# Alandroid/img-compression-mps

Hardware: AMD Instinct MI355X
Metric: Mvoxels/s compress+reconstruct, 256^3 fp32, bond chi=64; SSIM vs ref (higher is better)
Workload: dtype f32

## Files before the change

### img-compression-mps_amd/csrc/eig_tridiag.hip

```cpp
#include <math.h>
#include <stdlib.h>
#include <string.h>

#include <algorithm>
#include <atomic>
#include <map>
#include <mutex>
#include <vector>

#include "common.h"
#include "lanes.h"

namespace {
__device__ __forceinline__ double load_if(const double* p, bool ok) {
  const double v = *p;
  return ok ? v : 0.0;
}
}

namespace {

typedef double f64x4 __attribute__((ext_vector_type(4)));

constexpr int kTail = 128;
constexpr int kTailLd = 132;
constexpr int kMaxK = 128;
constexpr int kMaxN = 4096;

struct TrdDesc {
  const double* G_in;
  double* V_out;
  double* w_out;
  int n;
  int k;
  int status;
  int pad;
};

struct __attribute__((aligned(16))) TeamRec {
  double v;
  unsigned long long tag;
};

struct TeamSync {
  unsigned long long count;
  int abort;
  int pad[317];
};

struct TrdWork {
  double* A;
  double* Vh;
  double* y;
  double* xc;
  TeamRec* yr;
  TeamRec* xr;
  TeamSync* sync;
  double* tau;
  double* d;
  double* e;
  double* lam;
  double* mu;
  double* bound;
  double* Z;
  double* lu;
  unsigned char* piv;
  double* Tw;
  int64_t t_stride;
  double* yb;
  double* xb;
  double* band;
  double* qlog;
  int64_t q_stride;
  int tail_lower;
  int xcd_team, xcd_count;
  int xcd_pair;
  double* yrow;
  double* pv;
  double* pw;
  double* ypart;
  double* spart;
  double* ucol;
  double* napart;
  int pnl_blocks_max, pnl_tiles_max;
  long long* stamps;
  int n_max, lda, kp;
};

template <int STEPS>
__device__ __forceinline__ double fast_rsqrt(double x) {
  double y = __builtin_amdgcn_rsq(x);
#pragma unroll
  for (int i = 0; i < STEPS; ++i) y = y * fma(-0.5 * x * y, y, 1.5);
  return y;
}
template <int STEPS>
__device__ __forceinline__ double fast_rcp(double x) {
  double y = __builtin_amdgcn_rcp(x);
#pragma unroll
  for (int i = 0; i < STEPS; ++i) y = y * fma(-x, y, 2.0);
  return y;
}

__device__ __forceinline__ double wave_sum(double v) { return ndmps_lanes::sum_adjacent<64>(v); }

template <int NW>
// ... 18 lines not shown
  const double h2 = fma(alpha, alpha, sigma);
  const double rs = fast_rsqrt<2>(h2);
  const double nrm = h2 * rs;
  beta = alpha >= 0.0 ? -nrm : nrm;
  tau = (beta - alpha) * (alpha >= 0.0 ? -rs : rs);
  scale = fast_rcp<2>(alpha - beta);
}

__global__ void __launch_bounds__(256) trd_load_kernel(const TrdDesc* __restrict__ desc, TrdWork w) {
  const TrdDesc& d = desc[blockIdx.y];
  const int n = d.n, lda = w.lda;
  const double* G = d.G_in;
  double* A = w.A + (int64_t)blockIdx.y * w.n_max * lda;
  const int64_t total = (int64_t)n * lda;
  for (int64_t e = (int64_t)blockIdx.x * 256 + threadIdx.x; e < total; e += (int64_t)gridDim.x * 256) {
    const int r = (int)(e / lda), c = (int)(e % lda);
    A[e] = c < n ? 0.5 * (G[(int64_t)r * n + c] + G[(int64_t)c * n + r]) : 0.0;
  }
}

struct __attribute__((aligned(16))) RowVec {
  double vp, wp, vj, pad;
};

template <int NR, int CW>
__global__ void __launch_bounds__(256)
trd_column_kernel(const TrdDesc* __restrict__ desc, TrdWork w, int j) {
  constexpr int LPR = CW / 2;
  constexpr int RPW = 64 / LPR;
  constexpr int RPI = 4 * RPW;
  constexpr int PRE = 512 / RPI;
  const TrdDesc& d = desc[blockIdx.y];
  const int n = d.n;
  if (j >= n - kTail) return;
  const int c0 = blockIdx.x * CW;
  if (c0 >= n || c0 + CW <= j + 1) return;
  const int lda = w.lda;
  const int tid = threadIdx.x, lane = tid & 63, wave = tid >> 6;
  const int64_t b = blockIdx.y;
  double* A = w.A + b * w.n_max * lda;
  double* Vh = w.Vh + b * w.n_max * lda;
  double* ybuf = w.y + b * 2 * lda;
  extern __shared__ __attribute__((aligned(16))) double lds[];
  RowVec* rv = reinterpret_cast<RowVec*>(lds);
  __shared__ double red_a[4], red_b[4];
  __shared__ double part[4][CW];

  const int q = lane / LPR, p = lane % LPR;
  const int c = c0 + 2 * p;
  const bool col_ok = c < lda;
  const int first = j + 1 + RPW * wave + q;
  double2 a[PRE];
#pragma unroll
  for (int u = 0; u < PRE; ++u) {
    const int i = first + RPI * u;
    a[u] = (i < n && col_ok) ? *reinterpret_cast<const double2*>(A + (int64_t)i * lda + c) : make_double2(0.0, 0.0);
  }
  const double* rowj = A + (int64_t)j * lda;
  double yv[NR], vv[NR], rj[NR];
  double taup = 0.0, y_j = 0.0, y_j1 = 0.0, v_j1 = 0.0;
  const double r_j1 = rowj[j + 1];
  if (j >= 1) {
    const double* yprev = ybuf + ((j - 1) & 1) * lda;
    const double* vprev = Vh + (int64_t)(j - 1) * lda;
    taup = w.tau[b * w.n_max + j - 1];
    y_j = yprev[j];
    y_j1 = yprev[j + 1];
// ... 175 lines not shown
    member = blockIdx.x;
    team = blockIdx.y;
    return true;
  }
  const int L = blockIdx.x, full = w.xcd_count & ~7;
  if (L < full * w.xcd_team) {
    const int t = L >> 3;
    member = t % w.xcd_team;
    team = (t / w.xcd_team) * 8 + (L & 7);
    if (w.xcd_pair && ((t >> 5) & 1)) {
      const int blk = min(w.xcd_team, 32), pos = member % blk;
      member += blk - 1 - 2 * pos;
    }
  } else {
    const int r = w.xcd_count - full, l2 = L - full * w.xcd_team;
    member = l2 / r;
    team = full + l2 % r;
  }
  return true;
}

template <int NR, bool TAGGED, int CW = 32>
__global__ void __launch_bounds__(256, NR <= 4 ? 2 : 1)
trd_team_kernel(TrdDesc* __restrict__ desc, TrdWork w, int b0, unsigned epoch) {
  constexpr int MR = 256 * NR;
  constexpr int LPR = CW / 4;
  constexpr int RPW = 64 / LPR;
  constexpr int RPI = 4 * RPW;
  constexpr int NT = MR / RPI;
  int member, team;
  if (!team_place(w, member, team)) return;
  TrdDesc& d = desc[b0 + team];
  const int n = d.n;
  const int J = n - kTail;
  const int c0 = member * CW;
  if (J <= 0 || c0 >= n) return;
  const int nblk = (n + CW - 1) / CW;
  const int j_last = min(J - 1, c0 + CW - 2);
  const int lda = w.lda;
  const int tid = threadIdx.x, lane = tid & 63, wave = tid >> 6;
  const int64_t b = b0 + team;
  double* A = w.A + b * w.n_max * lda;
  double* Vh = w.Vh + b * w.n_max * lda;
  double* ybuf = w.y + b * 2 * lda;
  double* xc = w.xc + b * 2 * lda;
  TeamSync* sync = w.sync + b;
  TeamRec* yr = w.yr + b * 2 * lda;
  TeamRec* xr = w.xr + b * 2 * lda;
  const unsigned long long tag_base = (unsigned long long)epoch << 32;
  extern __shared__ __attribute__((aligned(32))) double team_dyn[];
  RowVec* rv = reinterpret_cast<RowVec*>(team_dyn);
  __shared__ double red_a[4], red_b[4];
  __shared__ double part[4][CW];
  __shared__ int go;

  const int q = lane % RPW, p = lane / RPW;
  const int c = c0 + 4 * p;
  const int row0 = RPW * wave + q;
  double a[NT][4];
#pragma unroll
  for (int u = 0; u < NT; ++u) {
    const int i = row0 + RPI * u;
    double2 lo = make_double2(0.0, 0.0), hi = lo;
    if (i < n) {
      if (c < lda) lo = *reinterpret_cast<const double2*>(A + (int64_t)i * lda + c);
      if (c + 2 < lda) hi = *reinterpret_cast<const double2*>(A + (int64_t)i * lda + c + 2);
    }
// ... 406 lines not shown
        sv.x -= me.vp * c0v.wp + me.wp * c0v.vp;
        sv.y -= me.vp * c1v.wp + me.wp * c1v.vp;
        acc = fma(sv.x, c0v.vj, acc);
        acc = fma(sv.y, c1v.vj, acc);
        *reinterpret_cast<double2*>(row + c) = sv;
      }
    }
    acc = ndmps_lanes::sum_adjacent<4>(acc);
    const double vjr = r < kTail ? cv[r].vj : 0.0;
    double dot = (t == 0 && r < m && r > jj) ? acc * vjr : 0.0;
    dot = wave_sum(dot);
    if (lane == 0) red_d[wave] = dot;
    __syncthreads();
    dot = 0.0;
#pragma unroll
    for (int x = 0; x < 8; ++x) dot += red_d[x];
    const double al = 0.5 * tau * tau * dot;
    if (t == 0 && r < m) {
      const double yr = r > jj ? acc : 0.0;
      cv[r].wp = tau * yr - al * vjr;
      cv[r].vp = vjr;
    }
    __syncthreads();
  }
  if (tid == 0) {
    const int jj = m - 1;
    dd[n - 1] = S[jj * kTailLd + jj] - 2.0 * cv[jj].vp * cv[jj].wp;
    ee[n - 1] = 0.0;
    tt[n - 1] = 0.0;
  }
  for (int i = tid; i < lda; i += 512) Vh[(int64_t)(n - 1) * lda + i] = 0.0;
}

__global__ void __launch_bounds__(512) trd_tail_reg_kernel(const TrdDesc* __restrict__ desc, TrdWork w) {
  const TrdDesc& d = desc[blockIdx.y];
  const int n = d.n;
  const int J = max(n - kTail, 0), m = n - J;
  const int lda = w.lda;
  const int tid = threadIdx.x, lane = tid & 63, wave = tid >> 6;
  const int64_t b = blockIdx.y;
  const double* A = w.A + b * w.n_max * lda;
  double* Vh = w.Vh + b * w.n_max * lda;
  const double* ybuf = w.y + b * 2 * lda;
  double* dd = w.d + b * w.n_max;
  double* ee = w.e + b * w.n_max;
  double* tt = w.tau + b * w.n_max;
  __shared__ RowVec cv[kTail];
  __shared__ double xrow[kTail];
  __shared__ double yv[kTail];
  __shared__ double red_s[8];

  for (int64_t e = tid; e < (int64_t)m * lda; e += 512) {
    const int i = (int)(e % lda);
    if (i < J || i >= n) Vh[(int64_t)J * lda + e] = 0.0;
  }
  if (J >= 1) {
    const double* yprev = ybuf + ((J - 1) & 1) * lda;
    const double* vprev = Vh + (int64_t)(J - 1) * lda;
    const double taup = tt[J - 1];
    double dot = 0.0, vv = 0.0, y0 = 0.0;
    if (tid < m) {
      vv = vprev[J + tid];
      y0 = yprev[J + tid];
      dot = y0 * vv;
    }
    dot = wave_sum(dot);
    if (lane == 0) red_s[wave] = dot;
    __syncthreads();
    dot = 0.0;
#pragma unroll
    for (int x = 0; x < 8; ++x) dot += red_s[x];
    const double al = 0.5 * taup * taup * dot;
    if (tid < kTail) {
      cv[tid].vp = tid < m ? vv : 0.0;
      cv[tid].wp = tid < m ? taup * y0 - al * vv : 0.0;
    }
  } else if (tid < kTail) {
    cv[tid].vp = 0.0;
    cv[tid].wp = 0.0;
  }
  __syncthreads();
  const int rg = tid >> 4, cg = tid & 15;
  double s[4][8];
#pragma unroll
  for (int a = 0; a < 4; ++a) {
    const int r = rg + 32 * a, gr = J + r;
    const double vpr = cv[r].vp, wpr = cv[r].wp;
#pragma unroll
    for (int q = 0; q < 8; ++q) {
      const int c = cg + 16 * q, gc = J + c;
      double v = 0.0;
      if (r < m && c < m) {
        const bool mirror = w.tail_lower && (gr >> 5) < (gc >> 5);
        const double av = mirror ? A[(int64_t)gc * lda + gr] : A[(int64_t)gr * lda + gc];
        v = av - (vpr * cv[c].wp + wpr * cv[c].vp);
      }
      s[a][q] = v;
    }
  }
  if (rg == 0) {
#pragma unroll
    for (int q = 0; q < 8; ++q) xrow[cg + 16 * q] = s[0][q];
  }
  __syncthreads();
  if (tid < kTail) {
    cv[tid].vp = 0.0;
    cv[tid].wp = 0.0;
    cv[tid].vj = 0.0;
  }
  __syncthreads();

  const int i0 = lane, i1 = lane + 64;
  double pv0 = 0.0, pv1 = 0.0, pw0 = 0.0, pw1 = 0.0;
  double tau_now = 0.0;
  auto pick = [&](double lo, double hi, int idx) {
    const double src = idx < 64 ? lo : hi;
    const long long bits = __double_as_longlong(src);
    const int l = __builtin_amdgcn_readlane((int)bits, idx & 63), h = __builtin_amdgcn_readlane((int)(bits >> 32), idx & 63);
    return __longlong_as_double(((long long)h << 32) | (unsigned)l);
  };
  for (int jj = 0; jj + 1 < m; ++jj) {
    const int j = J + jj;
    if (wave == 0) {
      const double vpj = pick(pv0, pv1, jj), wpj = pick(pw0, pw1, jj);
      double x0 = 0.0, x1 = 0.0;
      if (i0 < m) x0 = xrow[i0] - (vpj * pw0 + wpj * pv0);
      if (i1 < m) x1 = xrow[i1] - (vpj * pw1 + wpj * pv1);
      double sigma = (i0 > jj + 1 ? x0 * x0 : 0.0) + (i1 > jj + 1 ? x1 * x1 : 0.0);
      sigma = wave_sum(sigma);
      const double alpha = pick(x0, x1, jj + 1), djj = pick(x0, x1, jj);
      double beta, tau, scale;
      householder(alpha, sigma, beta, tau, scale);
      const double v0 = i0 > jj + 1 ? x0 * scale : (i0 == jj + 1 ? 1.0 : 0.0);
      const double v1 = i1 > jj + 1 ? x1 * scale : (i1 == jj + 1 ? 1.0 : 0.0);
      if (i0 < m) {
        cv[i0].vj = v0;
        Vh[(int64_t)j * lda + J + i0] = v0;
      }
      if (i1 < m) {
        cv[i1].vj = v1;
        Vh[(int64_t)j * lda + J + i1] = v1;
      }
      if (lane == 0) {
        dd[j] = djj;
        ee[j] = beta;
        tt[j] = tau;
      }
      tau_now = tau;
      pv0 = v0;
      pv1 = v1;
    }
    __syncthreads();
    double acc[4] = {0.0, 0.0, 0.0, 0.0};
    {
      const int q0 = (jj + 1) >> 4, a0 = (jj + 1) >> 5;
      double vpr[4], wpr[4];
#pragma unroll
      for (int a4 = 0; a4 < 4; ++a4) {
        vpr[a4] = cv[rg + 32 * a4].vp;
        wpr[a4] = cv[rg + 32 * a4].wp;
      }
#pragma unroll
      for (int h = 0; h < 2; ++h) {
        double vpc[4], wpc[4], vjc[4];
#pragma unroll
        for (int q = 0; q < 4; ++q) {
          const RowVec cr = cv[cg + 16 * (4 * h + q)];
          vpc[q] = cr.vp;
          wpc[q] = cr.wp;
          vjc[q] = cr.vj;
        }
#pragma unroll
        for (int a4 = 0; a4 < 4; ++a4) {
          if (a4 >= a0) {
#pragma unroll
            for (int q = 0; q < 4; ++q) {
              if (4 * h + q >= q0) {
                s[a4][4 * h + q] = fma(-vpr[a4], wpc[q], fma(-wpr[a4], vpc[q], s[a4][4 * h + q]));
                acc[a4] = fma(s[a4][4 * h + q], vjc[q], acc[a4]);
              }
            }
          }
        }
      }
      if (rg == ((jj + 1) & 31)) {
#define NDMPS_TAIL_PUT(AX) _Pragma("unroll") for (int q = 0; q < 8; ++q) xrow[cg + 16 * q] = s[AX][q];
        switch ((jj + 1) >> 5) {
          case 0: NDMPS_TAIL_PUT(0) break;
          case 1: NDMPS_TAIL_PUT(1) break;
          case 2: NDMPS_TAIL_PUT(2) break;
          default: NDMPS_TAIL_PUT(3) break;
        }
#undef NDMPS_TAIL_PUT
      }
    }
    const double y0 = ndmps_lanes::sum_adjacent<16>(acc[0]), y1 = ndmps_lanes::sum_adjacent<16>(acc[1]);
    const double y2 = ndmps_lanes::sum_adjacent<16>(acc[2]), y3 = ndmps_lanes::sum_adjacent<16>(acc[3]);
    if (cg < 4) {
      const int rr = rg + 32 * cg;
      const double yr = (cg & 2) ? ((cg & 1) ? y3 : y2) : ((cg & 1) ? y1 : y0);
      yv[rr] = rr > jj && rr < m ? yr : 0.0;
    }
    __syncthreads();
    if (wave == 0) {
      const double tau = tau_now;
      const double ya = yv[i0], yb = yv[i1];
      double dot = wave_sum(fma(ya, pv0, yb * pv1));
      const double al = 0.5 * tau * tau * dot;
      pw0 = tau * ya - al * pv0;
      pw1 = tau * yb - al * pv1;
      cv[i0].vp = pv0;
      cv[i0].wp = pw0;
      cv[i1].vp = pv1;
      cv[i1].wp = pw1;
    }
  }
  if (tid == 0) {
    const int jj = m - 1;
    dd[n - 1] = xrow[jj] - 2.0 * cv[jj].vp * cv[jj].wp;
    ee[n - 1] = 0.0;
    tt[n - 1] = 0.0;
  }
}

constexpr double kE2Floor = 0x1p-200;
__device__ __forceinline__ int sturm_count(const double2* __restrict__ de2, int n16, double x) {
  double pm = 0.0, pc = 1.0;
  int hp = 0;
  unsigned cnt = 0;
  for (int i0 = 0; i0 < n16; i0 += 16) {
    double2 v[16];
#pragma unroll
    for (int u = 0; u < 16; ++u) v[u] = de2[i0 + u];
#pragma unroll
    for (int u = 0; u < 16; ++u) {
      const double pn = fma(v[u].x - x, pc, -v[u].y * pm);
      const int hn = __double2hiint(pn);
      cnt += (unsigned)(hn ^ hp) >> 31;
      hp = hn;
      pm = pc;
      pc = pn;
      if ((u & 3) == 3) {
        const double mx = fmax(fabs(pm), fabs(pc));
        const int ex = mx > 0.0 ? ilogb(mx) : 0;
        pm = ldexp(pm, -ex);
        pc = ldexp(pc, -ex);
      }
// ... 899 lines not shown
    sync[base + t].abort = 0;
  }
}
__global__ void trd_setk_kernel(TrdDesc* __restrict__ desc, RankChunk chunk, int base, int count) {
  const int t = threadIdx.x;
  if (t < count) {
    desc[base + t].k = chunk.v[t];
    if (desc[base + t].status != 2) desc[base + t].status = 0;
  }
}
__global__ void trd_clear_status_kernel(TrdDesc* __restrict__ desc, int batch, TeamSync* __restrict__ sync) {
  const int b = blockIdx.x * blockDim.x + threadIdx.x;
  if (b < batch) {
    desc[b].status = 0;
    sync[b].count = 0;
    sync[b].abort = 0;
  }
}

#include "eig_band.inc"
#include "eig_sym.inc"
#include "eig_panel.inc"
#include "eig_wide.inc"

__global__ void trd_inject_abort_kernel(TrdDesc* __restrict__ desc, int batch) {
  const int b = blockIdx.x * blockDim.x + threadIdx.x;
  if (b < batch) desc[b].status = 2;
}

constexpr bool kTeamXcdDefault = true;
constexpr bool kSymDefault = false;
constexpr int kWideOrthoMinOrder = 1024;
constexpr int kWideOrthoMaxBatch = 2;
constexpr int kBandDefault = 0;

struct TrdLayout {
  int64_t n_max, lda, kp;
  int64_t off_a, off_vh, off_y, off_xc, off_yr, off_xr, off_sync, off_tau, off_d, off_e, off_lam, off_mu, off_bound, off_z, off_lu, off_piv, off_desc, off_desc2, off_stamps, off_tw, t_stride, off_yb, off_xb, off_band, off_qlog, q_stride, off_yrow, total;
  int64_t off_pv, off_pw, off_ypart, off_spart, off_ucol, off_napart, pnl_blocks, pnl_tiles;
  int64_t off_ws, off_wlinv, off_wgram, off_wt, wt_stride, kw, wgram_bytes, off_wpart, wpart_stride;
};

TrdLayout trd_layout(int64_t n_max, int64_t batch, int64_t k_max) {
  TrdLayout l;
  l.n_max = n_max;
  l.lda = ndmps::round_up(n_max, 2);
  l.kp = ndmps::round_up(std::max<int64_t>(k_max, 1), 16);
  int64_t used = 0;
  auto take = [&](int64_t bytes) {
    const int64_t off = ndmps::round_up(used, 256);
    used = off + bytes;
    return off;
  };
  l.off_a = take(batch * n_max * l.lda * 8);
  l.off_vh = take(batch * n_max * l.lda * 8);
  l.off_y = take(batch * 2 * l.lda * 8);
  l.off_xc = take(batch * 2 * l.lda * 8);
  l.off_yr = take(batch * 2 * l.lda * 16);
  l.off_xr = take(batch * 2 * l.lda * 16);
  l.off_sync = take(batch * (int64_t)sizeof(TeamSync));
  l.off_tau = take(batch * n_max * 8);
  l.off_d = take(batch * n_max * 8);
  l.off_e = take(batch * n_max * 8);
  l.off_lam = take(batch * n_max * 8);
  l.off_mu = take(batch * n_max * 8);
  l.off_bound = take(batch * 8);
// ... 42 lines not shown
  w.A = (double*)(base + l.off_a);
  w.Vh = (double*)(base + l.off_vh);
  w.y = (double*)(base + l.off_y);
  w.xc = (double*)(base + l.off_xc);
  w.yr = (TeamRec*)(base + l.off_yr);
  w.xr = (TeamRec*)(base + l.off_xr);
  w.sync = (TeamSync*)(base + l.off_sync);
  w.tau = (double*)(base + l.off_tau);
  w.d = (double*)(base + l.off_d);
  w.e = (double*)(base + l.off_e);
  w.lam = (double*)(base + l.off_lam);
  w.mu = (double*)(base + l.off_mu);
  w.bound = (double*)(base + l.off_bound);
  w.Z = (double*)(base + l.off_z);
  w.lu = (double*)(base + l.off_lu);
  w.piv = (unsigned char*)(base + l.off_piv);
  w.stamps = (long long*)(base + l.off_stamps);
  w.Tw = (double*)(base + l.off_tw);
  w.t_stride = l.t_stride;
  w.yb = (double*)(base + l.off_yb);
  w.xb = (double*)(base + l.off_xb);
  w.band = (double*)(base + l.off_band);
  w.qlog = (double*)(base + l.off_qlog);
  w.q_stride = l.q_stride;
  w.yrow = (double*)(base + l.off_yrow);
  w.pv = (double*)(base + l.off_pv);
  w.pw = (double*)(base + l.off_pw);
  w.ypart = (double*)(base + l.off_ypart);
  w.spart = (double*)(base + l.off_spart);
  w.ucol = (double*)(base + l.off_ucol);
  w.napart = (double*)(base + l.off_napart);
  w.pnl_blocks_max = (int)l.pnl_blocks;
  w.pnl_tiles_max = (int)l.pnl_tiles;
  w.tail_lower = 0;
  w.xcd_team = w.xcd_count = w.xcd_pair = 0;
  w.n_max = (int)l.n_max;
  w.lda = (int)l.lda;
  w.kp = (int)l.kp;
  return w;
}

constexpr int kInvitLdsMax = kMaxK * (kMaxK + 1) * 8;
constexpr size_t kTailLds = ((size_t)kTail * kTailLd + 4 * kTail) * sizeof(double);

thread_local int g_team_off = 0;
thread_local int g_team_streamed = 0;
std::atomic<long long> g_team_fallbacks{0};
std::atomic<int> g_inject_abort{0};


int trd_opt_in() {
  static std::mutex mu;
  static bool done[64] = {};
  int dev = 0;
  NDMPS_CHECK_HIP(hipGetDevice(&dev));
  std::lock_guard<std::mutex> lock(mu);
  if (dev < 0 || dev >= 64 || done[dev]) return NDMPS_OK;
  NDMPS_CHECK_HIP(hipFuncSetAttribute(reinterpret_cast<const void*>(&trd_tail_kernel),
                                      hipFuncAttributeMaxDynamicSharedMemorySize, (int)kTailLds));
  NDMPS_CHECK_HIP(hipFuncSetAttribute(reinterpret_cast<const void*>(&trd_team_kernel<8, true, 8>),
                                      hipFuncAttributeMaxDynamicSharedMemorySize, 2048 * (int)sizeof(RowVec)));
  NDMPS_CHECK_HIP(hipFuncSetAttribute(reinterpret_cast<const void*>(&trd_column_kernel<16, 32>),
                                      hipFuncAttributeMaxDynamicSharedMemorySize, kMaxN * (int)sizeof(RowVec)));
  NDMPS_CHECK_HIP(hipFuncSetAttribute(reinterpret_cast<const void*>(&trd_column_kernel<16, 8>),
                                      hipFuncAttributeMaxDynamicSharedMemorySize, kMaxN * (int)sizeof(RowVec)));
  NDMPS_CHECK_HIP(hipFuncSetAttribute(reinterpret_cast<const void*>(&trd_invit_kernel),
// ... 185 lines not shown
      const int nr = n_max <= 1024 ? 4 : 8;
      int slots = 0;
      NDMPS_TRY(team_slots(slots, nr));
      const int team_size = (int)ndmps::ceil_div(n_max, 8);
      const int per_launch = std::max(1, slots / team_size);
      w.tail_lower = 0;
      int inject = g_inject_abort.load();
      while (inject > 0 && !g_inject_abort.compare_exchange_weak(inject, inject - 1)) {
      }
      if (inject > 0) {
        hipLaunchKernelGGL(trd_inject_abort_kernel, dim3((batch + 63) / 64), dim3(64), 0, s, desc, batch);
        return NDMPS_OK;
      }
      return team_launch(s, [&]() {
        for (int b0 = 0; b0 < batch; b0 += per_launch) {
          const unsigned epoch = g_team_epoch.fetch_add(1);
          const dim3 grid((unsigned)team_size, (unsigned)std::min(per_launch, batch - b0));
          TrdWork wl = w;
          wl.xcd_count = 0;
          if (nr == 4) hipLaunchKernelGGL((trd_team_kernel<4, true, 8>), grid, dim3(256), 1024 * sizeof(RowVec), s, desc, wl, b0, epoch);
          else hipLaunchKernelGGL((trd_team_kernel<8, true, 8>), grid, dim3(256), 2048 * sizeof(RowVec), s, desc, wl, b0, epoch);
        }
      });
    }
    int slots = 0;
    NDMPS_TRY(team_slots(slots));
    const bool streamed = g_team_streamed && !getenv("NDMPS_TRD_TEAM_NARROW");
    const bool narrow_team = (int64_t)batch * ndmps::ceil_div(n_max, 8) <= (streamed ? slots / 2 : slots) &&
                             !getenv("NDMPS_TRD_TEAM_WIDE");
    const char* sym_env = getenv("NDMPS_TRD_SYM");
    const bool sym = !narrow_team && n_max <= 512 && (sym_env ? atoi(sym_env) != 0 : kSymDefault) &&
                     (int64_t)batch * ndmps::ceil_div(n_max, 32) > slots / 2;
    w.tail_lower = sym ? 1 : 0;
    const int team_size = sym ? (int)ndmps::ceil_div(ndmps::ceil_div(n_max, 32), 2) : (int)ndmps::ceil_div(n_max, narrow_team ? 8 : 32);
    const bool half_launches = getenv("NDMPS_TRD_TEAM_HALF") != nullptr && !narrow_team && !sym;
    const int per_launch = std::max(1, (half_launches ? slots / 2 : slots) / team_size);
    const char* xcd_env = getenv("NDMPS_TRD_XCD");
    const bool xcd_placed = xcd_env ? atoi(xcd_env) != 0 : kTeamXcdDefault;
    int inject = g_inject_abort.load();
    while (inject > 0 && !g_inject_abort.compare_exchange_weak(inject, inject - 1)) {
    }
    if (inject > 0) {
      hipLaunchKernelGGL(trd_inject_abort_kernel, dim3((batch + 63) / 64), dim3(64), 0, s, desc, batch);
    } else
    NDMPS_TRY(team_launch(s, [&]() {
      for (int b0 = 0; b0 < batch; b0 += per_launch) {
        const unsigned epoch = g_team_epoch.fetch_add(1);
        const int count = std::min(per_launch, batch - b0);
        TrdWork wl = w;
        dim3 grid((unsigned)team_size, (unsigned)count);
        if (xcd_placed) {
          wl.xcd_team = team_size;
          wl.xcd_count = count;
          const bool pairable = 32 % team_size == 0 || team_size % 32 == 0;
          wl.xcd_pair = sym || !pairable ? 0 : getenv("NDMPS_TRD_PAIR") ? atoi(getenv("NDMPS_TRD_PAIR")) : 1;
          grid = dim3((unsigned)(team_size * count));
        }
        if (sym) hipLaunchKernelGGL(trd_sym_kernel, grid, dim3(256), 0, s, desc, wl, b0);
        else if (narrow_team) hipLaunchKernelGGL((trd_team_kernel<2, true, 8>), grid, dim3(256), 512 * sizeof(RowVec), s, desc, wl, b0, epoch);
        else hipLaunchKernelGGL((trd_team_kernel<2, false>), grid, dim3(256), 512 * sizeof(RowVec), s, desc, wl, b0, epoch);
      }
    }, (int64_t)std::min(per_launch, batch) * team_size <= slots / 2));
  return NDMPS_OK;
}

int trd_reduce_and_values(int batch, const int64_t* h_n, int64_t n_max, int64_t k_max, const TrdLayout& l, const TrdWork& w_in,
                          TrdDesc* desc, hipStream_t s) {
  TrdWork w = w_in;
  const unsigned B = (unsigned)batch;
  const int load_grid = (int)std::min<int64_t>(ndmps::ceil_div(n_max * l.lda, 256), 512);
  hipLaunchKernelGGL(trd_load_kernel, dim3(load_grid, B), dim3(256), 0, s, desc, w);
  const bool narrow = (int64_t)batch * ndmps::ceil_div(n_max, 8) <= 2 * ndmps::kNumCU && !getenv("NDMPS_TRD_WIDE");
  const int W = (int)ndmps::ceil_div(n_max, narrow ? 8 : 32);
  const size_t col_lds = (size_t)n_max * sizeof(RowVec);
  void (*column)(const TrdDesc*, TrdWork, int);
  if (narrow)
    column = n_max <= 512    ? trd_column_kernel<2, 8>
             : n_max <= 1024 ? trd_column_kernel<4, 8>
             : n_max <= 2048 ? trd_column_kernel<8, 8>
                             : trd_column_kernel<16, 8>;
  else
    column = n_max <= 512    ? trd_column_kernel<2, 32>
             : n_max <= 1024 ? trd_column_kernel<4, 32>
             : n_max <= 2048 ? trd_column_kernel<8, 32>
                             : trd_column_kernel<16, 32>;
  const int bw = band_width_for(n_max);
  route_store(w_in.A, bw);
  const bool team = !bw && n_max <= 512 && n_max > kTail && !getenv("NDMPS_TRD_NO_TEAM") && !g_team_off;
  if (bw) {
    int slots = 0;
    NDMPS_TRY(team_slots(slots));
    const int team_size = (int)ndmps::ceil_div(n_max, 32);
    const int per_launch = std::max(1, slots / team_size);
    int inject = g_inject_abort.load();
    while (inject > 0 && !g_inject_abort.compare_exchange_weak(inject, inject - 1)) {
    }
    void* span = ndmps::span_begin(s);
    if (inject > 0) {
      hipLaunchKernelGGL(trd_inject_abort_kernel, dim3((batch + 63) / 64), dim3(64), 0, s, desc, batch);
    } else {
      NDMPS_TRY(team_launch(s, [&]() {
        for (int b0 = 0; b0 < batch; b0 += per_launch) {
          const dim3 grid((unsigned)team_size, (unsigned)std::min(per_launch, batch - b0));
          if (bw == 2) hipLaunchKernelGGL(trd_band_kernel<2>, grid, dim3(256), 0, s, desc, w, b0);
          else hipLaunchKernelGGL(trd_band_kernel<4>, grid, dim3(256), 0, s, desc, w, b0);
        }
      }));
    }
    int64_t bytes = 0;
    for (int b = 0; b < batch; ++b) bytes += 2 * 8 * h_n[b] * h_n[b];
    ndmps::span_end(span, s, ndmps::kSpanTridiagTeam, 1, bytes);
    const size_t chase_lds = (size_t)n_max * 2 * bw * sizeof(double);
    if (bw == 2) hipLaunchKernelGGL(trd_chase_kernel<2>, dim3(1, B), dim3(1024), chase_lds, s, desc, w);
    else hipLaunchKernelGGL(trd_chase_kernel<4>, dim3(1, B), dim3(1024), chase_lds, s, desc, w);
    const int kk = (int)std::min(k_max, n_max);
    hipLaunchKernelGGL(trd_bisect_kernel, dim3(ndmps::ceil_div(kk, 4), B), dim3(256),
                       (size_t)ndmps::round_up(n_max, 16) * 16, s, desc, w, kk);
    NDMPS_LAUNCH_CHECK();
    return NDMPS_OK;
  }
  const bool team_on = !bw && !g_team_off && !getenv("NDMPS_TRD_NO_TEAM");
// ... 49 lines not shown
    }
    NDMPS_TRY(pnl_run(seq, batch, h_n, n_max, tail_cols, desc, w, s));
    if (hybrid) {
      const int64_t J0 = n_max - hybrid;
      TrdDesc* sub = (TrdDesc*)((char*)w_in.A - l.off_a + l.off_desc2);
      hipLaunchKernelGGL(pnl_mirror_kernel, dim3(256, B), dim3(256), 0, s, w, (int)n_max, hybrid);
      hipLaunchKernelGGL(pnl_subdesc_kernel, dim3((batch + 63) / 64), dim3(64), 0, s, (const TrdDesc*)desc, sub, batch, hybrid);
      TrdWork v = w;
      v.A = w.A + J0 * l.lda + J0;
      v.Vh = w.Vh + J0 * l.lda + J0;
      v.y = w.y + J0;
      v.tau = w.tau + J0;
      v.d = w.d + J0;
      v.e = w.e + J0;
      NDMPS_TRY(trd_team_reduce(batch, hybrid, sub, v, s));
      hipLaunchKernelGGL(pnl_substatus_kernel, dim3((batch + 63) / 64), dim3(64), 0, s, desc, (const TrdDesc*)sub, batch);
      w.tail_lower = 0;
    } else {
      NDMPS_CHECK_HIP(hipMemsetAsync(w.y, 0, (size_t)batch * 2 * l.lda * 8, s));
    }
    ndmps::span_end(span, s, ndmps::kSpanTridiagPanel, (int64_t)seq.size(), span_bytes);
  } else {
    for (int j = 0; j < n_max - kTail; ++j) {
      hipLaunchKernelGGL(column, dim3(W, B), dim3(256), col_lds, s, desc, w, j);
      if (span)
        for (int b = 0; b < batch; ++b)
          if (j < h_n[b] - kTail) span_bytes += 2 * 8 * (h_n[b] - j - 1) * (h_n[b] - j - 1);
    }
    ndmps::span_end(span, s, ndmps::kSpanTridiagColumns, std::max<int64_t>(n_max - kTail, 0), span_bytes);
  }
  const char* tail_env = getenv("NDMPS_TRD_TAIL");
  const bool tail_regs = tail_env ? !strcmp(tail_env, "regs") : batch < 16;
  void* tail_span = ndmps::span_begin(s);
  if (tail_regs) hipLaunchKernelGGL(trd_tail_reg_kernel, dim3(1, B), dim3(512), 0, s, desc, w);
  else hipLaunchKernelGGL(trd_tail_kernel, dim3(1, B), dim3(512), kTailLds, s, desc, w);
  const int kk = (int)std::min(k_max, n_max);
  hipLaunchKernelGGL(trd_bisect_kernel, dim3(ndmps::ceil_div(kk, 4), B), dim3(256),
                     (size_t)ndmps::round_up(n_max, 16) * 16, s, desc, w, kk);
  ndmps::span_end(tail_span, s, ndmps::kSpanTridiagTail, 2, 0);
  NDMPS_LAUNCH_CHECK();
  return NDMPS_OK;
}

}

extern "C" int64_t ndmps_potrf_scratch_elems(int64_t n) {
  const int64_t kw = ndmps::round_up(std::max<int64_t>(n, 1), kWB);
  return kw * kw + 64;
}
extern "C" int ndmps_potrf_lower_f64(double* d_S, int64_t n, double* d_scratch, int* h_status, ndmps_stream_t stream) {
  NDMPS_REQUIRE(d_S && d_scratch && h_status && n >= 1 && n <= 32768, "bad Cholesky argument");
  NDMPS_TRY(trd_opt_in());
  hipStream_t s = (hipStream_t)stream;
  const int k = (int)n, kw = (int)ndmps::round_up(n, kWB), nblk = kw / kWB;
  double* linv = d_scratch;
  TrdDesc* d_flag = reinterpret_cast<TrdDesc*>(d_scratch + (int64_t)kw * kw);
  NDMPS_CHECK_HIP(hipMemsetAsync(d_flag, 0, sizeof(TrdDesc), s));
  for (int pb = 0; pb < nblk; ++pb) {
    const int p = kWB * pb, below = nblk - pb - 1;
    hipLaunchKernelGGL(wide_chol_diag_kernel, dim3(1), dim3(512), (size_t)2 * kWB * kWLd * sizeof(double), s, d_S, k, linv, kw, k, p,
                       d_flag);
    if (below > 0) {
      hipLaunchKernelGGL(wide_chol_panel_kernel, dim3((unsigned)below), dim3(256), 0, s, d_S, k, (const double*)linv, kw, k, p);
      hipLaunchKernelGGL(wide_chol_trail_kernel, dim3((unsigned)(below * (below + 1) / 2)), dim3(256), 0, s, d_S, k, k, p);
    }
  }
  hipLaunchKernelGGL(wide_zero_upper_kernel, dim3((unsigned)std::min<int64_t>(ndmps::ceil_div(n * n, 256), 2048)), dim3(256), 0, s,
// ... 348 lines not shown
```

### img-compression-mps_amd/csrc/tt.hip

```cpp
#include <math.h>
#include <stdlib.h>

#include <algorithm>
#include <vector>

#include "common.h"
#include "trunc.h"

namespace {

constexpr double kCutoffFloor = 1e-6;
constexpr double kCutoffFloorF64 = 1e-8;
template <typename T>
constexpr double cutoff_floor() { return sizeof(T) == 8 ? kCutoffFloorF64 : kCutoffFloor; }
constexpr double kSweepEigTol = 1e-13;

inline double sweep_eig_tol(bool f64_storage = false) {
  const char* e = getenv("NDMPS_SWEEP_EIG_TOL");
  if (e) {
    const double v = atof(e);
    if (v >= 1e-16 && v <= 1e-6) return v;
  }
  return f64_storage ? 1e-15 : kSweepEigTol;
}
// ... 97 lines not shown
scale_cols_to_f32_kernel(const double* __restrict__ M, int64_t rows, int64_t ldm, int64_t k,
                         const double* __restrict__ sigma, double power, T* __restrict__ out) {
  scale_cols_body(M, rows, ldm, k, sigma, power, out);
}
template <typename T>
__global__ void __launch_bounds__(256)
scale_rows_to_f32_kernel(const double* __restrict__ M, int64_t k, int64_t n, const double* __restrict__ sigma,
                         double power, T* __restrict__ out) {
  scale_rows_body(M, k, n, sigma, power, out);
}
__global__ void __launch_bounds__(256) sqrt_clamp_kernel(const double* __restrict__ w, int64_t n, double* s) {
  sqrt_clamp_body(w, n, s);
}

__global__ void __launch_bounds__(256)
scale_cols_sqrt_kernel(double* __restrict__ M, int64_t rows, int64_t cols, const double* __restrict__ w,
                       double rel_zero = 0.0) {
  const double zero = rel_zero * fmax(fmax(w[0], w[cols - 1]), 0.0);
  const int64_t total = rows * cols;
  for (int64_t e = (int64_t)blockIdx.x * 256 + threadIdx.x; e < total; e += (int64_t)gridDim.x * 256) {
    const double we = w[e % cols];
    M[e] *= we > zero ? sqrt(we) : 0.0;
  }
}

constexpr int kSmallBatch = 64;
struct BatchOps {
  const void* in[kSmallBatch];
  void* out[kSmallBatch];
};
template <typename T>
__global__ void __launch_bounds__(256) f32_to_f64_batched_kernel(BatchOps ops, int64_t n, double* __restrict__ y, int64_t y_stride) {
  f32_to_f64_body(static_cast<const T*>(ops.in[blockIdx.y]), n, y + (int64_t)blockIdx.y * y_stride);
}
template <typename T>
__global__ void __launch_bounds__(256)
core_from_vectors_batched_kernel(const double* __restrict__ V, int64_t v_stride, int64_t n, int64_t k, BatchOps ops) {
  core_from_vectors_body(V + (int64_t)blockIdx.y * v_stride, n, k, static_cast<T*>(ops.out[blockIdx.y]));
}
__global__ void __launch_bounds__(256)
sqrt_clamp_batched_kernel(const double* __restrict__ w, int64_t stride, int64_t n, double* __restrict__ sg) {
  sqrt_clamp_body(w + (int64_t)blockIdx.y * stride, n, sg + (int64_t)blockIdx.y * stride);
}
template <typename T>
__global__ void __launch_bounds__(256)
scale_cols_to_f32_batched_kernel(const double* __restrict__ M, int64_t m_stride, int64_t rows, int64_t ldm, int64_t k,
                                 const double* __restrict__ sigma, int64_t s_stride, double power, BatchOps ops) {
  scale_cols_body(M + (int64_t)blockIdx.y * m_stride, rows, ldm, k, sigma + (int64_t)blockIdx.y * s_stride, power,
                  static_cast<T*>(ops.out[blockIdx.y]));
}
template <typename T>
__global__ void __launch_bounds__(256)
scale_rows_to_f32_batched_kernel(const double* __restrict__ M, int64_t m_stride, int64_t k, int64_t n,
                                 const double* __restrict__ sigma, int64_t s_stride, double power, BatchOps ops) {
  scale_rows_body(M + (int64_t)blockIdx.y * m_stride, k, n, sigma + (int64_t)blockIdx.y * s_stride, power,
                  static_cast<T*>(ops.out[blockIdx.y]));
}

struct MergeRanks {
  int k_right[64];
  int k_here[64];
};

__global__ void __launch_bounds__(256)
merge_stage1_kernel(const double* __restrict__ Gtop, int64_t stride_top, int n_top, const double* __restrict__ W,
                    int64_t stride_w, int ldw, double* __restrict__ T, int64_t stride_t, int n_i, int n_right,
// ... 871 lines not shown
    hipLaunchKernelGGL(scale_cols_to_f32_batched_kernel<T>, dim3(grid1d(m * k), batch), dim3(256), 0, s, ws.V,
                       sq, m, m, k, ws.sig, lay.small_max, 1.0, carry_out);
    NDMPS_LAUNCH_CHECK();
    NDMPS_TRY(ndmps_dgemm_batched(batch, 1, 0, k, n, m, pv.data(), m, pa.data(), n, pu.data(), n, s));
    hipLaunchKernelGGL(scale_rows_to_f32_batched_kernel<T>, dim3(grid1d(k * n), batch), dim3(256), 0, s,
                       ws.UtA, lay.wide_elems, k, n, ws.sig, lay.small_max, -1.0,
                       cores_out);
    NDMPS_LAUNCH_CHECK();
    return NDMPS_OK;
  }

  int core_and_carry_volume(int i, int b) {
    const int64_t n = h_dims[i] * chi_r[b], m = cur_elems[b] / n, small = eig_n[b], k = kept[b];
    const double* sigb = ws.sig + (int64_t)b * lay.small_max;
    if (n <= m) {
      hipLaunchKernelGGL(core_from_vectors_kernel<T>, dim3(grid1d(k * n)), dim3(256), 0, s, Vb(b), n, k,
                         core(b, i));
      NDMPS_LAUNCH_CHECK();
      return gemm_T(1, m, k, n, cur[b], core(b, i), n, nxt[b], ws.tws, lay.transpose_bytes, s);
    }
    hipLaunchKernelGGL(sqrt_clamp_kernel, dim3(grid1d(small)), dim3(256), 0, s, ws.w + (int64_t)b * lay.small_max,
                       small, ws.sig + (int64_t)b * lay.small_max);
    hipLaunchKernelGGL(scale_cols_to_f32_kernel<T>, dim3(grid1d(m * k)), dim3(256), 0, s, Vb(b), m, m, k, sigb,
                       1.0, nxt[b]);
    NDMPS_LAUNCH_CHECK();
    NDMPS_TRY(ndmps_dgemm(1, 0, k, n, m, Vb(b), m, ws.A64 + (int64_t)b * lay.wide_elems, n, ws.UtA, n, s));
    hipLaunchKernelGGL(scale_rows_to_f32_kernel<T>, dim3(grid1d(k * n)), dim3(256), 0, s, ws.UtA, k, n, sigb,
                       -1.0, core(b, i));
    NDMPS_LAUNCH_CHECK();
    return NDMPS_OK;
  }

  int finish() {
    for (int b = 0; b < batch; ++b)
      NDMPS_CHECK_HIP(hipMemcpyAsync(core(b, 0), cur[b], cur_elems[b] * sizeof(T), hipMemcpyDeviceToDevice, s));
    if (!lay.device_rank || L <= 1) {
      if (async) {
        ndmps::set_error("an asynchronous sweep needs ranks decided on the device (ndmps_tt_sweep_pads_cores) and more than one site");
        return NDMPS_EINVAL;
      }
      NDMPS_CHECK_HIP(hipStreamSynchronize(s));
      return NDMPS_OK;
    }
    const size_t n_i = (size_t)2 * L * batch, n_s = (size_t)L * batch * lay.spec_stride;
    std::vector<int> host_i(async ? 0 : n_i);
    std::vector<double> host_s(async ? 0 : n_s);
    if (async) NDMPS_REQUIRE(async->h_ranks && (async->h_spec || n_s == 0), "asynchronous sweep without its host buffers");
    int* dst_i = async ? async->h_ranks : host_i.data();
    double* dst_s = async ? async->h_spec : host_s.data();
    NDMPS_CHECK_HIP(hipMemcpyAsync(dst_i, ws.d_ranks, n_i * sizeof(int), hipMemcpyDeviceToHost, s));
    if (n_s) NDMPS_CHECK_HIP(hipMemcpyAsync(dst_s, ws.d_spec, n_s * sizeof(double), hipMemcpyDeviceToHost, s));
    if (async) return NDMPS_OK;
    NDMPS_CHECK_HIP(hipStreamSynchronize(s));
    return sweep_collect(batch, L, lay.spec_stride, dst_i, n_s ? dst_s : nullptr, h_bonds_out, h_spectra, h_spec_offsets);
  }
};

template <typename T>
int sweep_impl(int batch, T* const* h_dense, int L, const int64_t* h_dims, double cutoff, int64_t max_bond,
               T* const* h_cores, const int64_t* h_core_offsets, int64_t* h_bonds_out, double* h_spectra,
               const int64_t* h_spec_offsets, void* d_ws, int64_t ws_bytes, ndmps_stream_t stream,
               const SweepSource* src = nullptr, const SweepAsync* async = nullptr) {
  Sweep<T> sw{batch, h_dense, L, h_dims, cutoff, max_bond, h_cores, h_core_offsets, h_bonds_out, h_spectra,
              h_spec_offsets, d_ws, ws_bytes, (hipStream_t)stream, src, async};
  NDMPS_TRY(sw.prepare());
  int i = L - 1;
  if (sw.lay.merge_from < L) {
    NDMPS_TRY(sw.merged_run());
// ... 747 lines not shown
```

Measured before the change: 42440.

## Template tail tridiagonal kernel on order and batch final core copies

The register-resident tail tridiagonalization kernel is templated on the trailing order (128 or 192), with a runtime tail width in the work struct. The wider tail is selected only when the NDMPS_TRD_TAIL_COLS environment variable asks for it. Separately, the per-batch device-to-device memcpy calls in finish() are replaced by one batched copy kernel launch per 64 items, which cuts launch and API overhead. The tail kernel also now reads previous v/w from shared memory instead of registers, which may add shared-memory traffic.

Measured after the change: 42510, median of 3. Within noise of the previous version (+0.2%).

```diff
diff --git a/img-compression-mps_amd/csrc/eig_tridiag.hip b/img-compression-mps_amd/csrc/eig_tridiag.hip
--- a/img-compression-mps_amd/csrc/eig_tridiag.hip
+++ b/img-compression-mps_amd/csrc/eig_tridiag.hip
@@ -23,6 +23,7 @@
 typedef double f64x4 __attribute__((ext_vector_type(4)));
 
 constexpr int kTail = 128;
+constexpr int kTailWide = 192;
 constexpr int kTailLd = 132;
 constexpr int kMaxK = 128;
 constexpr int kMaxN = 4096;
@@ -72,6 +73,7 @@
   double* band;
   double* qlog;
   int64_t q_stride;
+  int tail;
   int tail_lower;
   int xcd_team, xcd_count;
   int xcd_pair;
@@ -156,7 +158,7 @@
   constexpr int PRE = 512 / RPI;
   const TrdDesc& d = desc[blockIdx.y];
   const int n = d.n;
-  if (j >= n - kTail) return;
+  if (j >= n - w.tail) return;
   const int c0 = blockIdx.x * CW;
   if (c0 >= n || c0 + CW <= j + 1) return;
   const int lda = w.lda;
@@ -398,7 +400,7 @@
   if (!team_place(w, member, team)) return;
   TrdDesc& d = desc[b0 + team];
   const int n = d.n;
-  const int J = n - kTail;
+  const int J = n - w.tail;
   const int c0 = member * CW;
   if (J <= 0 || c0 >= n) return;
   const int nblk = (n + CW - 1) / CW;
@@ -871,10 +873,17 @@
   for (int i = tid; i < lda; i += 512) Vh[(int64_t)(n - 1) * lda + i] = 0.0;
 }
 
-__global__ void __launch_bounds__(512) trd_tail_reg_kernel(const TrdDesc* __restrict__ desc, TrdWork w) {
+template <int M>
+__global__ void __launch_bounds__(4 * M) trd_tail_reg_kernel(const TrdDesc* __restrict__ desc, TrdWork w) {
+  static_assert(M == 128 || M == 192, "trailing order 128 or 192");
+  constexpr int NTH = 4 * M;
+  constexpr int RB = M / 4;
+  constexpr int NQ = M / 16;
+  constexpr int NP = M / 64;
+  constexpr int NWV = NTH / 64;
   const TrdDesc& d = desc[blockIdx.y];
   const int n = d.n;
-  const int J = max(n - kTail, 0), m = n - J;
+  const int J = max(n - M, 0), m = n - J;
   const int lda = w.lda;
   const int tid = threadIdx.x, lane = tid & 63, wave = tid >> 6;
   const int64_t b = blockIdx.y;
@@ -884,14 +893,14 @@
   double* dd = w.d + b * w.n_max;
   double* ee = w.e + b * w.n_max;
   double* tt = w.tau + b * w.n_max;
-  __shared__ RowVec cv[kTail];
-  __shared__ double xrow[kTail];
-  __shared__ double yv[kTail];
-  __shared__ double red_s[8];
-
-  for (int64_t e = tid; e < (int64_t)m * lda; e += 512) {
+  __shared__ RowVec cv[M];
+  __shared__ double xrow[M];
+  __shared__ double yv[M];
+  __shared__ double red_s[NWV];
+
+  for (int64_t e = tid; e < (int64_t)m * lda; e += NTH) {
     const int i = (int)(e % lda);
-    if (i < J || i >= n) Vh[(int64_t)J * lda + e] = 0.0;
+    if (i < J || i >= n || e >= (int64_t)(m - 1) * lda) Vh[(int64_t)J * lda + e] = 0.0;
   }
   if (J >= 1) {
     const double* yprev = ybuf + ((J - 1) & 1) * lda;
@@ -908,25 +917,25 @@
     __syncthreads();
     dot = 0.0;
 #pragma unroll
-    for (int x = 0; x < 8; ++x) dot += red_s[x];
+    for (int x = 0; x < NWV; ++x) dot += red_s[x];
     const double al = 0.5 * taup * taup * dot;
-    if (tid < kTail) {
+    if (tid < M) {
       cv[tid].vp = tid < m ? vv : 0.0;
       cv[tid].wp = tid < m ? taup * y0 - al * vv : 0.0;
     }
-  } else if (tid < kTail) {
+  } else if (tid < M) {
     cv[tid].vp = 0.0;
     cv[tid].wp = 0.0;
   }
   __syncthreads();
   const int rg = tid >> 4, cg = tid & 15;
-  double s[4][8];
+  double s[4][NQ];
 #pragma unroll
   for (int a = 0; a < 4; ++a) {
-    const int r = rg + 32 * a, gr = J + r;
+    const int r = rg + RB * a, gr = J + r;
     const double vpr = cv[r].vp, wpr = cv[r].wp;
 #pragma unroll
-    for (int q = 0; q < 8; ++q) {
+    for (int q = 0; q < NQ; ++q) {
       const int c = cg + 16 * q, gc = J + c;
       double v = 0.0;
       if (r < m && c < m) {
@@ -939,46 +948,49 @@
   }
   if (rg == 0) {
 #pragma unroll
-    for (int q = 0; q < 8; ++q) xrow[cg + 16 * q] = s[0][q];
+    for (int q = 0; q < NQ; ++q) xrow[cg + 16 * q] = s[0][q];
   }
   __syncthreads();
-  if (tid < kTail) {
+  if (tid < M) {
     cv[tid].vp = 0.0;
     cv[tid].wp = 0.0;
     cv[tid].vj = 0.0;
   }
   __syncthreads();
 
-  const int i0 = lane, i1 = lane + 64;
-  double pv0 = 0.0, pv1 = 0.0, pw0 = 0.0, pw1 = 0.0;
   double tau_now = 0.0;
-  auto pick = [&](double lo, double hi, int idx) {
-    const double src = idx < 64 ? lo : hi;
+  auto pick3 = [](double x0, double x1, double x2, int idx) {
+    double src = (idx >> 6) == 1 ? x1 : x0;
+    if constexpr (NP > 2) src = (idx >> 6) == 2 ? x2 : src;
     const long long bits = __double_as_longlong(src);
     const int l = __builtin_amdgcn_readlane((int)bits, idx & 63), h = __builtin_amdgcn_readlane((int)(bits >> 32), idx & 63);
     return __longlong_as_double(((long long)h << 32) | (unsigned)l);
   };
+  auto pick = [&](const double (&x)[NP], int idx) { return pick3(x[0], x[1], x[NP - 1], idx); };
   for (int jj = 0; jj + 1 < m; ++jj) {
     const int j = J + jj;
     if (wave == 0) {
-      const double vpj = pick(pv0, pv1, jj), wpj = pick(pw0, pw1, jj);
-      double x0 = 0.0, x1 = 0.0;
-      if (i0 < m) x0 = xrow[i0] - (vpj * pw0 + wpj * pv0);
-      if (i1 < m) x1 = xrow[i1] - (vpj * pw1 + wpj * pv1);
-      double sigma = (i0 > jj + 1 ? x0 * x0 : 0.0) + (i1 > jj + 1 ? x1 * x1 : 0.0);
+      const double vpj = cv[jj].vp, wpj = cv[jj].wp;
+      double x[NP];
+      double sigma = 0.0;
+#pragma unroll
+      for (int p = 0; p < NP; ++p) {
+        const int i = lane + 64 * p;
+        x[p] = i < m ? xrow[i] - (vpj * cv[i].wp + wpj * cv[i].vp) : 0.0;
+        sigma += i > jj + 1 ? x[p] * x[p] : 0.0;
+      }
       sigma = wave_sum(sigma);
-      const double alpha = pick(x0, x1, jj + 1), djj = pick(x0, x1, jj);
+      const double alpha = pick(x, jj + 1), djj = pick(x, jj);
       double beta, tau, scale;
       householder(alpha, sigma, beta, tau, scale);
-      const double v0 = i0 > jj + 1 ? x0 * scale : (i0 == jj + 1 ? 1.0 : 0.0);
-      const double v1 = i1 > jj + 1 ? x1 * scale : (i1 == jj + 1 ? 1.0 : 0.0);
-      if (i0 < m) {
-        cv[i0].vj = v0;
-        Vh[(int64_t)j * lda + J + i0] = v0;
-      }
-      if (i1 < m) {
-        cv[i1].vj = v1;
-        Vh[(int64_t)j * lda + J + i1] = v1;
+#pragma unroll
+      for (int p = 0; p < NP; ++p) {
+        const int i = lane + 64 * p;
+        const double v = i > jj + 1 ? x[p] * scale : (i == jj + 1 ? 1.0 : 0.0);
+        if (i < m) {
+          cv[i].vj = v;
+          Vh[(int64_t)j * lda + J + i] = v;
+        }
       }
       if (lane == 0) {
         dd[j] = djj;
@@ -986,21 +998,19 @@
         tt[j] = tau;
       }
       tau_now = tau;
-      pv0 = v0;
-      pv1 = v1;
     }
     __syncthreads();
     double acc[4] = {0.0, 0.0, 0.0, 0.0};
     {
-      const int q0 = (jj + 1) >> 4, a0 = (jj + 1) >> 5;
+      const int q0 = (jj + 1) >> 4, a0 = (jj + 1) / RB;
       double vpr[4], wpr[4];
 #pragma unroll
       for (int a4 = 0; a4 < 4; ++a4) {
-        vpr[a4] = cv[rg + 32 * a4].vp;
-        wpr[a4] = cv[rg + 32 * a4].wp;
-      }
-#pragma unroll
-      for (int h = 0; h < 2; ++h) {
+        vpr[a4] = cv[rg + RB * a4].vp;
+        wpr[a4] = cv[rg + RB * a4].wp;
+      }
+#pragma unroll
+      for (int h = 0; h < NQ / 4; ++h) {
         double vpc[4], wpc[4], vjc[4];
 #pragma unroll
         for (int q = 0; q < 4; ++q) {
@@ -1022,9 +1032,9 @@
           }
         }
       }
-      if (rg == ((jj + 1) & 31)) {
-#define NDMPS_TAIL_PUT(AX) _Pragma("unroll") for (int q = 0; q < 8; ++q) xrow[cg + 16 * q] = s[AX][q];
-        switch ((jj + 1) >> 5) {
+      if (rg == (jj + 1) % RB) {
+#define NDMPS_TAIL_PUT(AX) _Pragma("unroll") for (int q = 0; q < NQ; ++q) xrow[cg + 16 * q] = s[AX][q];
+        switch ((jj + 1) / RB) {
           case 0: NDMPS_TAIL_PUT(0) break;
           case 1: NDMPS_TAIL_PUT(1) break;
           case 2: NDMPS_TAIL_PUT(2) break;
@@ -1036,22 +1046,28 @@
     const double y0 = ndmps_lanes::sum_adjacent<16>(acc[0]), y1 = ndmps_lanes::sum_adjacent<16>(acc[1]);
     const double y2 = ndmps_lanes::sum_adjacent<16>(acc[2]), y3 = ndmps_lanes::sum_adjacent<16>(acc[3]);
     if (cg < 4) {
-      const int rr = rg + 32 * cg;
+      const int rr = rg + RB * cg;
       const double yr = (cg & 2) ? ((cg & 1) ? y3 : y2) : ((cg & 1) ? y1 : y0);
       yv[rr] = rr > jj && rr < m ? yr : 0.0;
     }
     __syncthreads();
     if (wave == 0) {
       const double tau = tau_now;
-      const double ya = yv[i0], yb = yv[i1];
-      double dot = wave_sum(fma(ya, pv0, yb * pv1));
+      double ys[NP], pv[NP];
+      double dot = 0.0;
+#pragma unroll
+      for (int p = 0; p < NP; ++p) {
+        ys[p] = yv[lane + 64 * p];
+        pv[p] = cv[lane + 64 * p].vj;
+        dot = fma(ys[p], pv[p], dot);
+      }
+      dot = wave_sum(dot);
       const double al = 0.5 * tau * tau * dot;
-      pw0 = tau * ya - al * pv0;
-      pw1 = tau * yb - al * pv1;
-      cv[i0].vp = pv0;
-      cv[i0].wp = pw0;
-      cv[i1].vp = pv1;
-      cv[i1].wp = pw1;
+#pragma unroll
+      for (int p = 0; p < NP; ++p) {
+        cv[lane + 64 * p].vp = pv[p];
+        cv[lane + 64 * p].wp = tau * ys[p] - al * pv[p];
+      }
     }
   }
   if (tid == 0) {
@@ -2017,6 +2033,7 @@
 constexpr bool kSymDefault = false;
 constexpr int kWideOrthoMinOrder = 1024;
 constexpr int kWideOrthoMaxBatch = 2;
+constexpr int kTailColsDefault = kTail;
 constexpr int kBandDefault = 0;
 
 struct TrdLayout {
@@ -2125,6 +2142,7 @@
   w.napart = (double*)(base + l.off_napart);
   w.pnl_blocks_max = (int)l.pnl_blocks;
   w.pnl_tiles_max = (int)l.pnl_tiles;
+  w.tail = kTail;
   w.tail_lower = 0;
   w.xcd_team = w.xcd_count = w.xcd_pair = 0;
   w.n_max = (int)l.n_max;
@@ -2376,6 +2394,7 @@
     const bool sym = !narrow_team && n_max <= 512 && (sym_env ? atoi(sym_env) != 0 : kSymDefault) &&
                      (int64_t)batch * ndmps::ceil_div(n_max, 32) > slots / 2;
     w.tail_lower = sym ? 1 : 0;
+    if (sym) w.tail = kTail;
     const int team_size = sym ? (int)ndmps::ceil_div(ndmps::ceil_div(n_max, 32), 2) : (int)ndmps::ceil_div(n_max, narrow_team ? 8 : 32);
     const bool half_launches = getenv("NDMPS_TRD_TEAM_HALF") != nullptr && !narrow_team && !sym;
     const int per_launch = std::max(1, (half_launches ? slots / 2 : slots) / team_size);
@@ -2431,6 +2450,9 @@
   const int bw = band_width_for(n_max);
   route_store(w_in.A, bw);
   const bool team = !bw && n_max <= 512 && n_max > kTail && !getenv("NDMPS_TRD_NO_TEAM") && !g_team_off;
+  const char* cols_env = getenv("NDMPS_TRD_TAIL_COLS");
+  const int cols = cols_env ? atoi(cols_env) : kTailColsDefault;
+  w.tail = team && n_max > kTailWide && cols == kTailWide ? kTailWide : kTail;
   if (bw) {
     int slots = 0;
     NDMPS_TRY(team_slots(slots));
@@ -2546,7 +2568,8 @@
   const char* tail_env = getenv("NDMPS_TRD_TAIL");
   const bool tail_regs = tail_env ? !strcmp(tail_env, "regs") : batch < 16;
   void* tail_span = ndmps::span_begin(s);
-  if (tail_regs) hipLaunchKernelGGL(trd_tail_reg_kernel, dim3(1, B), dim3(512), 0, s, desc, w);
+  if (w.tail == kTailWide) hipLaunchKernelGGL(trd_tail_reg_kernel<kTailWide>, dim3(1, B), dim3(4 * kTailWide), 0, s, desc, w);
+  else if (tail_regs) hipLaunchKernelGGL(trd_tail_reg_kernel<kTail>, dim3(1, B), dim3(4 * kTail), 0, s, desc, w);
   else hipLaunchKernelGGL(trd_tail_kernel, dim3(1, B), dim3(512), kTailLds, s, desc, w);
   const int kk = (int)std::min(k_max, n_max);
   hipLaunchKernelGGL(trd_bisect_kernel, dim3(ndmps::ceil_div(kk, 4), B), dim3(256),
diff --git a/img-compression-mps_amd/csrc/tt.hip b/img-compression-mps_amd/csrc/tt.hip
--- a/img-compression-mps_amd/csrc/tt.hip
+++ b/img-compression-mps_amd/csrc/tt.hip
@@ -153,6 +153,16 @@
 template <typename T>
 __global__ void __launch_bounds__(256) f32_to_f64_batched_kernel(BatchOps ops, int64_t n, double* __restrict__ y, int64_t y_stride) {
   f32_to_f64_body(static_cast<const T*>(ops.in[blockIdx.y]), n, y + (int64_t)blockIdx.y * y_stride);
+}
+struct BatchCounts {
+  int64_t n[kSmallBatch];
+};
+template <typename T>
+__global__ void __launch_bounds__(256) copy_batched_kernel(BatchOps ops, BatchCounts cnt) {
+  const T* in = static_cast<const T*>(ops.in[blockIdx.y]);
+  T* out = static_cast<T*>(ops.out[blockIdx.y]);
+  const int64_t n = cnt.n[blockIdx.y];
+  for (int64_t e = (int64_t)blockIdx.x * 256 + threadIdx.x; e < n; e += (int64_t)gridDim.x * 256) out[e] = in[e];
 }
 template <typename T>
 __global__ void __launch_bounds__(256)
@@ -1090,8 +1100,20 @@
   }
 
   int finish() {
-    for (int b = 0; b < batch; ++b)
-      NDMPS_CHECK_HIP(hipMemcpyAsync(core(b, 0), cur[b], cur_elems[b] * sizeof(T), hipMemcpyDeviceToDevice, s));
+    for (int base = 0; base < batch; base += kSmallBatch) {
+      const int count = std::min(kSmallBatch, batch - base);
+      BatchOps ops;
+      BatchCounts cnt;
+      int64_t biggest = 1;
+      for (int t = 0; t < count; ++t) {
+        ops.in[t] = cur[base + t];
+        ops.out[t] = core(base + t, 0);
+        cnt.n[t] = cur_elems[base + t];
+        biggest = std::max(biggest, cnt.n[t]);
+      }
+      hipLaunchKernelGGL(copy_batched_kernel<T>, dim3(grid1d(biggest), count), dim3(256), 0, s, ops, cnt);
+    }
+    NDMPS_LAUNCH_CHECK();
     if (!lay.device_rank || L <= 1) {
       if (async) {
         ndmps::set_error("an asynchronous sweep needs ranks decided on the device (ndmps_tt_sweep_pads_cores) and more than one site");
```
